# wangheda/youtube-8m

Measured on AMD Instinct MI355X. Metric: training videos/sec, higher is better.
Workload: dtype f32; 1 GPU; BASELINE configs[3]: LstmModel (2 x BasicLSTMCell(1024), dynamic_rnn over F=300) on raw uint8 [B,300,1152] frames + MoeModel head (2 mixtures, V=4716), fp32 training step (fwd+bwd+clip+Adam); per_gpu_batch=128, global_batch=128, frames=300, parallelism=dp1, params=113902808

## Files before the change

### include/yt8m_hip.h

```cpp
#ifndef YT8M_HIP_H
#define YT8M_HIP_H
#include <stdint.h>

#ifdef __cplusplus
extern "C" {
#endif

typedef void* yt8m_stream_t;

enum yt8m_status { YT8M_OK = 0, YT8M_E_BADARG = -1, YT8M_E_SHAPE = -2, YT8M_E_HIP = -3, YT8M_E_RCCL = -4 };
enum yt8m_label_dtype { YT8M_LABEL_U8 = 0, YT8M_LABEL_F32 = 1 };

int yt8m_abi_version(void);
const char* yt8m_last_error(void);
const char* yt8m_built_arch(void);

int yt8m_prof_enable(int on);
int yt8m_prof_reset(void);
int yt8m_prof_get(int family, int64_t* launches, double* total_ms);
int yt8m_prof_get_flops(int family, double* flops);
int yt8m_prof_get_bytes(int family, double* bytes);

int yt8m_probe_mfma_f32(int iters, int blocks, float* sink, yt8m_stream_t stream);
int yt8m_probe_mfma_bf16(int iters, int blocks, int random_operands, float* sink, yt8m_stream_t stream);
// ... 23 lines not shown
                          int64_t workspace_bytes, yt8m_stream_t stream);
int yt8m_gemm_bf16_nt_grouped(int nprob, const yt8m_gemm_problem* probs, void* workspace, int64_t workspace_bytes,
                              yt8m_stream_t stream);
int64_t yt8m_x3_image_bytes(int64_t rows, int64_t K);
int yt8m_x3_split(const float* src, int64_t R, int64_t C, int64_t ld, float scale, void* plain, void* trans, yt8m_stream_t stream);
int yt8m_gemm_x3_nt_grouped(int nprob, const yt8m_gemm_problem* probs, void* workspace, int64_t workspace_bytes,
                            yt8m_stream_t stream);
int yt8m_h2_split(const float* src, int64_t R, int64_t C, int64_t ld, float scale, const float* dscale, void* plain, void* trans,
                  float* colpart, yt8m_stream_t stream);
int yt8m_h2_absmax(const float* src, int64_t R, int64_t C, int64_t ld, void* word, yt8m_stream_t stream);
int yt8m_h2_degraded(uint64_t* counts, int reset, yt8m_stream_t stream);
int yt8m_h2_split_dropout(const float* src, int64_t R, int64_t C, float scale, const float* dscale, void* plain, void* trans,
                          float keep_prob, uint64_t seed, int64_t offset, yt8m_stream_t stream);
int yt8m_h2_split_rowmax(const float* src, int64_t R, int64_t C, int64_t ld, const void* rowmax, float* inv, void* plain,
                         yt8m_stream_t stream);
int yt8m_h2_split_ex(const float* src, int64_t R, int64_t C, int64_t ld, float scale, const void* dscale, const float* rowscale, void* plain,
                     void* trans, void* trans_scaled, float* colpart, float* colpart_scaled, yt8m_stream_t stream);
int yt8m_gemm_h1x2_nt_ex(int64_t M, int64_t N, int64_t K, const void* A1, int64_t ska, const void* B2, int64_t skb, float* C, int64_t ldc,
                         const float* bias, float alpha, const void* dsb, const float* rowscale, const float* colsum, float colsum_scale,
                         float beta, void* workspace, int64_t workspace_bytes, yt8m_stream_t stream);
int yt8m_h2_rowscales(const float* src, int64_t R, int64_t C, int64_t ld, float* S, float* inv, yt8m_stream_t stream);
int yt8m_h2_split_rows(const float* src, int64_t R, int64_t C, int64_t ld, const float* S, void* plain, yt8m_stream_t stream);
int yt8m_gemm_h2_nt_ex(int64_t M, int64_t N, int64_t K, const void* A2, int64_t ska, const void* B2, int64_t skb, float* C, int64_t ldc,
                       const float* bias, float alpha, const void* dsa, const void* dsb, const float* rowscale, float beta, void* workspace,
                       int64_t workspace_bytes, yt8m_stream_t stream);
int yt8m_timepool_max_f32(const float* y, int64_t F, int64_t B, int64_t N, int64_t ldy, float* out, int32_t* idx, int64_t ldo,
                          yt8m_stream_t stream);
int yt8m_timepool_shiftmax_f32(const float* z, int64_t F, int64_t B, int64_t ldz, int nfilt, const int32_t* fs, const int32_t* ncol, float* out,
                               int32_t* idx, int64_t ldo, yt8m_stream_t stream);
int yt8m_u8_cnn_pool_dw(const uint8_t* q, const float* r_tm, const int32_t* idx, const float* g, int64_t ldg, int64_t B, int64_t F, int64_t D,
// ... 282 lines not shown
  int64_t B, F, D, H;
  int32_t L;
  int32_t input_u8;
  float forget_bias;
  int32_t fwd_chunks;
  int32_t bwd_chunks;
  int32_t need_dx;
  float input_keep_prob;
  int32_t reserved0;
  uint64_t dropout_seed[8];
} yt8m_lstm_stack_desc;
int yt8m_lstm_stack_supported(const yt8m_lstm_stack_desc* desc);
int64_t yt8m_lstm_stack_tape_bytes(const yt8m_lstm_stack_desc* desc);
int64_t yt8m_lstm_stack_scratch_bytes(const yt8m_lstm_stack_desc* desc);
int yt8m_lstm_stack_partition(const yt8m_lstm_stack_desc* desc, int* fwd_chunks, int* bwd_chunks);
int yt8m_lstm_stack_streams(int L, yt8m_stream_t* layer_streams, yt8m_stream_t* wgrad_stream);
int yt8m_lstm_stack_fwd(const yt8m_lstm_stack_desc* desc, const void* x, const int32_t* num_frames, const float* const* W,
                        const float* const* b, void* tape, int64_t tape_bytes, void* scratch, int64_t scratch_bytes,
                        yt8m_stream_t stream);
int yt8m_lstm_stack_view(const yt8m_lstm_stack_desc* desc, void* tape, int layer, int which, float** out);
int yt8m_lstm_stack_bwd(const yt8m_lstm_stack_desc* desc, const void* x, const int32_t* num_frames, const float* const* W, void* tape,
                        int64_t tape_bytes, void* scratch, int64_t scratch_bytes, const float* dout_top,
                        const float* const* dc_final, const float* const* dh_final, float* const* dW, float* const* db,
                        const float* beta_W, const float* beta_b, float* dx, yt8m_stream_t stream);
int yt8m_lstm_stack_status(const yt8m_lstm_stack_desc* desc, void* scratch, yt8m_stream_t stream);
int yt8m_lstm_stack_layer_done_wait(int layer, yt8m_stream_t stream);
int yt8m_lstm_stack_use_streams(int set, int* previous);
typedef void (*yt8m_stream_hook)(void* user, yt8m_stream_t stream);
int yt8m_lstm_stack_set_prep_hook(yt8m_stream_hook hook, void* user);
typedef struct yt8m_opt_ranges {
// ... 166 lines not shown
```

### youtube-8m_amd/_lib.py

```python
import ctypes
import os

_HERE = os.path.dirname(os.path.abspath(__file__))
LIB_PATH = os.environ.get("YT8M_LIB", os.path.join(_HERE, "libyt8m_hip.so"))

c_void_p, c_int, c_int64, c_float, c_double = ctypes.c_void_p, ctypes.c_int, ctypes.c_int64, ctypes.c_float, ctypes.c_double
P = c_void_p

class GemmProblem(ctypes.Structure):
    _fields_ = [("M", c_int64), ("N", c_int64), ("K", c_int64), ("A", c_void_p), ("lda", c_int64), ("B", c_void_p),
                ("ldb", c_int64), ("C", c_void_p), ("ldc", c_int64), ("bias", c_void_p), ("beta", c_float)]


STREAM_HOOK = ctypes.CFUNCTYPE(None, ctypes.c_void_p, ctypes.c_void_p)


class PersistBwdImages(ctypes.Structure):
    _fields_ = [("plain", ctypes.c_void_p), ("trans", ctypes.c_void_p), ("trans_scaled", ctypes.c_void_p), ("rowscale", ctypes.c_void_p),
                ("colpart", ctypes.c_void_p), ("colpart_scaled", ctypes.c_void_p)]


class LstmStackDesc(ctypes.Structure):
    _fields_ = [("B", c_int64), ("F", c_int64), ("D", c_int64), ("H", c_int64), ("L", ctypes.c_int32), ("input_u8", ctypes.c_int32),
                ("forget_bias", c_float), ("fwd_chunks", ctypes.c_int32), ("bwd_chunks", ctypes.c_int32), ("need_dx", ctypes.c_int32),
# ... 159 lines not shown
    "yt8m_lstm_persist_set_cus": (c_int, [c_int, c_int]),
    "yt8m_lstm_persist_get_cus": (c_int, [ctypes.POINTER(c_int), ctypes.POINTER(c_int)]),
    "yt8m_lstm_persist_status": (c_int, [P, P]),
    "yt8m_lstm_persist_reserve_cus": (c_int, [c_int, ctypes.POINTER(c_int)]),
    "yt8m_lstm_persist_debug_fault": (c_int, [P, P]),
    "yt8m_lstm_persist_fwd": (c_int, [P, P, c_int64, P, P, P, P, c_int64, c_int64, c_int64, c_int64, c_float, P, c_int64, P]),
    "yt8m_lstm_persist_fwd_bf16": (c_int, [P, P, c_int64, P, P, P, P, c_int64, c_int64, c_int64, c_int64, c_float, P, c_int64, P]),
    "yt8m_lstm_persist_bwd_supported": (c_int, [c_int64, c_int64]),
    "yt8m_lstm_persist_bwd": (c_int, [P, P, c_int64, P, P, P, P, c_int, P, P, c_int64, c_int64, c_int64, c_int64, P, c_int64, P]),
    "yt8m_lstm_persist_bwd_bf16": (c_int, [P, P, c_int64, P, P, P, P, c_int, P, P, c_int64, c_int64, c_int64, c_int64, P, c_int64, P]),
    "yt8m_lstm_persist_fwd_h2": (c_int, [P, P, c_int64, P, P, P, P, c_int64, c_int64, c_int64, c_int64, c_float, P, P, c_int64, P]),
    "yt8m_lstm_persist_bwd_h2": (c_int, [P, P, c_int64, P, P, P, P, c_int, P, P, c_int64, c_int64, c_int64, c_int64, P, P, c_int64, P]),
    "yt8m_lstm_persist_bwd_on_f16_pipe": (c_int, [c_int64, c_int64]),
    "yt8m_lstm_persist_bwd_ex": (c_int, [P, P, c_int64, P, P, P, P, c_int, P, c_int64, c_int64, c_int64, c_int64, P, P, P, P, c_int64, P]),
    "yt8m_h2_split_rowmax": (c_int, [P, c_int64, c_int64, c_int64, P, P, P, P]),
    "yt8m_lstm_persist_bwd_images_rows": (c_int, [c_int64, c_int64]),
    "yt8m_lstm_persist_bwd_images": (c_int, [P, P, c_int64, P, P, P, P, c_int, P, c_int64, c_int64, c_int64, c_int64, P, c_int64, P, P]),
    "yt8m_lstm_packed_floats": (c_int64, [c_int64, c_int64]),
    "yt8m_lstm_pack": (c_int, [P, c_int64, c_int64, P, P, P]),
    "yt8m_lstm_steps_fwd": (c_int, [P, P, c_int64, P, P, P, P, P, c_int64, c_int64, c_int64, c_int64, c_float, P, c_int64, P]),
    "yt8m_lstm_steps_bwd": (c_int, [P, P, c_int64, P, P, P, P, P, c_int, P, c_int64, c_int64, c_int64, c_int64, P, c_int64, P]),
    "yt8m_lstm_layer_bwd": (c_int, [P, P, c_int64, P, P, P, P, P, P, P, c_int64, c_int64, c_int64, P, c_int64, P]),
    "yt8m_attn_softmax_fwd": (c_int, [P, P, P, c_int64, c_int64, c_int64, P]),
    "yt8m_attn_softmax_bwd": (c_int, [P, P, P, P, c_int64, c_int64, c_int64, P]),
    "yt8m_softmax_rows_fwd": (c_int, [P, P, P, c_int64, c_int64, c_int64, P]),
    "yt8m_softmax_rows_bwd": (c_int, [P, P, P, P, c_int64, c_int64, c_int64, P]),
    "yt8m_netvlad_supported": (c_int, [c_int64, c_int64, c_int64, c_int64]),
    "yt8m_netvlad_single_pass": (c_int, [c_int64, c_int64, c_int64, c_int64]),
    "yt8m_netvlad_set_single": (c_int, [c_int]),
    "yt8m_netvlad_workspace_bytes": (c_int64, [c_int64, c_int64, c_int64, c_int64]),
# ... 135 lines not shown
```

### youtube-8m_amd/csrc/gemm_x3.hip

```cpp
#include "common.h"
#include "x3_image.h"
#include "philox.h"
#include <type_traits>
#include <algorithm>
#include <mutex>
#include <stdlib.h>

namespace {

constexpr int TM = 256, TN = 256;
constexpr int PLANE_F = 256 * 8;
constexpr int OP_F = 3 * PLANE_F;
constexpr int NST = 3;
using yt8m_x3::RG_F;
using yt8m_x3::store_block;

typedef float f32x16 __attribute__((ext_vector_type(16)));
typedef __bf16 bf16x8 __attribute__((ext_vector_type(8)));

struct XArgs {
  const float* A;
  const float* B;
  float* C;
  const float* bias;
// ... 1027 lines not shown
        else store_block<NP>(v, trans + ((int64_t)(row >> 5) * KB + kb) * (NP * RG_F), row);
      }
      if (trans_s) {
#pragma unroll
        for (int j = 0; j < 16; ++j) {
          const int r = r0 + blk * 16 + j;
          v[j] *= r < R ? rowscale[r] : 0.f;
        }
        if constexpr (NP == 2) yt8m_x3::store_block_h2(v, trans_s + ((int64_t)(row >> 5) * KB + kb) * (NP * RG_F), row);
        else store_block<NP>(v, trans_s + ((int64_t)(row >> 5) * KB + kb) * (NP * RG_F), row);
      }
    }
  }
}

}

using namespace yt8m;

namespace {
constexpr size_t H2_DEGRADED_BYTES = 256 * 128;
unsigned long long* h2_degraded_words() {
  static std::mutex mu;
  static unsigned long long* words[64] = {};
  static bool tried[64] = {};
  int dev = 0;
  if (hipGetDevice(&dev) != hipSuccess || dev < 0 || dev >= 64) return nullptr;
  std::lock_guard<std::mutex> lk(mu);
  if (!tried[dev]) {
    tried[dev] = true;
// ... 174 lines not shown
                     (float*)nullptr, 1.0f, (const float*)nullptr, (float*)nullptr, (float*)nullptr, (float*)nullptr, (const float*)nullptr, S,
                     (const unsigned*)nullptr, (float*)nullptr, h2_degraded_words());
  return launch_status("x3_split_kernel<2>");
}
extern "C" int yt8m_h2_split_rowmax(const float* src, int64_t R, int64_t C, int64_t ld, const void* rowmax, float* inv, void* plain,
                                    yt8m_stream_t stream) {
  YT8M_REQUIRE(src && rowmax && inv && plain && R >= 1 && C >= 1 && ld >= C && R < (1LL << 31) && C < (1LL << 31), YT8M_E_BADARG, "bad arguments");
  YT8M_REQUIRE((reinterpret_cast<uintptr_t>(plain) & 15) == 0, YT8M_E_BADARG, "images must be 16-byte aligned");
  dim3 grid((unsigned)((C + 63) / 64), (unsigned)((R + 63) / 64));
  YT8M_REQUIRE(grid.y < 65536, YT8M_E_BADARG, "too many rows for one split launch");
  ProfScope prof(F_ELEMENTWISE, as_stream(stream));
  hipLaunchKernelGGL(x3_split_kernel<2>, grid, dim3(256), 0, as_stream(stream), src, ld, (int)R, (int)C, static_cast<float*>(plain),
                     (float*)nullptr, 1.0f, (const float*)nullptr, (float*)nullptr, (float*)nullptr, (float*)nullptr, (const float*)nullptr,
                     (const float*)nullptr, static_cast<const unsigned*>(rowmax), inv, h2_degraded_words());
  return launch_status("x3_split_kernel<2>");
}
extern "C" int yt8m_gemm_h2_nt_ex(int64_t M, int64_t N, int64_t K, const void* A2, int64_t ska, const void* B2, int64_t skb, float* C,
                                  int64_t ldc, const float* bias, float alpha, const void* dsa, const void* dsb, const float* rowscale,
                                  float beta, void* workspace, int64_t workspace_bytes, yt8m_stream_t stream);

extern "C" int yt8m_h2_absmax(const float* src, int64_t R, int64_t C, int64_t ld, void* word, yt8m_stream_t stream) {
  YT8M_REQUIRE(src && word && R >= 1 && C >= 1 && ld >= C && R < (1LL << 31) && C < (1LL << 31), YT8M_E_BADARG, "bad arguments");
  const int64_t n = R * C;
  const unsigned blocks = (unsigned)std::min<int64_t>(2048, (n + 4095) / 4096);
  ProfScope prof(F_ELEMENTWISE, as_stream(stream));
  hipLaunchKernelGGL(h2_absmax_kernel, dim3(blocks), dim3(256), 0, as_stream(stream), src, ld, (int)R, (int)C, static_cast<unsigned*>(word));
  return launch_status("h2_absmax_kernel");
}

extern "C" int yt8m_x3_split_ex(const float* src, int64_t R, int64_t C, int64_t ld, float scale, const float* rowscale, void* plain,
// ... 281 lines not shown
```

### youtube-8m_amd/csrc/lstm_stack.hip

```cpp
#include <stdlib.h>
#include <algorithm>
#include <mutex>
#include <vector>
#include "common.h"

using namespace yt8m;

namespace {

constexpr int MAXL = 8, MAXP = 64;
constexpr int MAXBP = 62;
constexpr float U8_ALPHA = 4.0f / 255.0f;
constexpr float U8_BETA = 128.0f * (4.0f / 255.0f) + (4.0f / 512.0f - 2.0f);
constexpr int64_t X3_MIN_ROWS = 1024;
constexpr int64_t STEP_IMAGES_MAX_BYTES = 8LL << 30;
constexpr float H2_S = 8192.0f;

int64_t up256(int64_t v) { return (v + 255) / 256 * 256; }

int knob(const char* name, int dflt) { const char* v = getenv(name); return v ? atoi(v) : dflt; }

struct Part { int64_t t0, T; };
int chunks(int64_t F, int n, Part* out) {
  if (n < 1) n = 1;
// ... 7 lines not shown

struct Plan {
  int64_t B, F, D, H, FB;
  int L, u8, need_dx;
  int bf16;
  int nf, nb;
  Part fp[MAXP], bp[MAXP];
  int64_t z[MAXL], cs[MAXL], hs[MAXL], out[MAXL], rrow, tape_bytes;
  int64_t pws[MAXL], pws_bytes;
  int64_t gws[MAXL + 1], gws_bytes;
  int64_t gwx[MAXL], gws2;
  int64_t qimg, w3t, wcs, wxt3[MAXL], xi[MAXL];
  int64_t dz[MAXL], dbuf[MAXL], work[MAXL];
  int64_t dz3[MAXL], wx3[MAXL], dzT3[MAXL], dzT3s, csr, dbdummy;
  int64_t xT[MAXL], hT[MAXL];
  int64_t cpart[MAXL], cparts;
  bool colparts;
  int img_rows;
  int h2;
  int64_t hsc;
  int64_t hx0;
  int64_t hrow, hrow_stride;
  float keep;
  uint64_t seed[MAXL];
  int emit_max;
  int64_t rmax, rmax_stride;
  int64_t cimg[MAXL], cimgs;
  int64_t scratch_bytes;
};

// ... 62 lines not shown
  p.pws_bytes = up256(pb);
  o = 0;
  for (int l = 0; l < p.L; ++l) { p.pws[l] = o; o += p.pws_bytes; }
  p.gws_bytes = up256(yt8m_gemm_workspace_bytes());
  for (int l = 0; l <= p.L; ++l) { p.gws[l] = o; o += p.gws_bytes; }
  for (int l = 0; l < p.L; ++l) { p.gwx[l] = o; o += p.gws_bytes; }
  p.gws2 = o; o += p.gws_bytes;
  auto ib = [&](int64_t rows, int64_t K) { return p.bf16 ? x1_bytes(rows, K) : x3_bytes(rows, K); };
  const int64_t H4 = 4 * p.H;
  p.qimg = o; o += p.u8 ? up256(x1_bytes(p.FB, p.D)) : 0;
  p.w3t = o; o += p.u8 ? up256(ib(H4, p.D)) : 0;
  p.wcs = o; o += up256(H4 * 4);
  int64_t fmax = 0, bmax = 0;
  for (int c = 0; c < p.nf; ++c) fmax = std::max(fmax, p.fp[c].T * p.B);
  for (int c = 0; c < p.nb; ++c) bmax = std::max(bmax, p.bp[c].T * p.B);
  for (int l = 0; l < p.L; ++l) {
    const int64_t Din = l ? p.H : p.D;
    const bool x1 = l == 0 && p.u8;
    p.wxt3[l] = o; o += x1 ? 0 : up256(ib(H4, Din));
    p.xi[l] = o; o += x1 ? 0 : up256(ib(fmax, Din));
    p.dz[l] = o; o += up256(FBH * 4 * 4);
    p.dbuf[l] = o; o += l + 1 < p.L ? up256(FBH * 4) : 0;
    p.work[l] = o; o += up256(4 * BH * 4);
    const bool dxl = l > 0 || p.need_dx;
    p.dz3[l] = o; o += dxl ? up256(ib(bmax, H4)) : 0;
    p.wx3[l] = o; o += dxl ? up256(ib(Din, H4)) : 0;
    p.xT[l] = o; o += x1 ? up256(x1_bytes(p.D, p.FB)) : up256(ib(Din, p.FB));
    p.hT[l] = o; o += up256(ib(p.H, p.FB));
  }
  p.h2 = (knob("YT8M_STACK_H2", 1) && !p.bf16) ? 1 : 0;
  p.keep = (d->input_keep_prob > 0.f && d->input_keep_prob < 1.f) ? d->input_keep_prob : 0.f;
  for (int l = 0; l < MAXL; ++l) p.seed[l] = d->dropout_seed[l];
  if (d->input_keep_prob < 0.f || d->input_keep_prob > 1.f) return "input_keep_prob must be in [0, 1]";
  if (p.keep > 0.f && (p.u8 || !p.h2 || p.keep < 0.3f || (p.D % 4) != 0 || (p.H % 4) != 0))
    return "input dropout: float input, f16 product forms (YT8M_STACK_H2), keep_prob >= 0.3, D % 4 == 0";
  p.img_rows = (knob("YT8M_STACK_FUSED_IMAGES", 0) && !p.bf16 && !p.h2) ? yt8m_lstm_persist_bwd_images_rows(p.B, p.H) : 0;
  const int64_t trows = p.img_rows ? p.FB : bmax;
  for (int l = 0; l < p.L; ++l) { p.dzT3[l] = o; o += up256(ib(H4, trows)); }
  p.dzT3s = o; o += p.u8 ? up256(ib(H4, trows)) : 0;
  const int64_t ci = p.img_rows ? up256((int64_t)p.img_rows * MAXP * 2 * H4 * 4) : 0;
  for (int l = 0; l < p.L; ++l) { p.cimg[l] = o; o += ci; }
  p.cimgs = o; o += p.u8 ? ci : 0;
  p.csr = o; o += up256(H4 * 4);
  p.dbdummy = o; o += up256(H4 * 4);
  p.hsc = o; o += 256 * MAXL;
  p.hx0 = o; o += 256;
  p.hrow_stride = up256(bmax * 4);
  p.hrow = o; o += p.h2 ? p.hrow_stride * 2 * MAXL : 0;
  p.emit_max = (p.h2 && knob("YT8M_STACK_DZ_MAXIMA", 1) && yt8m_lstm_persist_bwd_images_rows(p.B, p.H) > 0 && per_step && p.nb <= 61) ? 1 : 0;
  p.rmax_stride = up256(p.FB * 4);
  p.rmax = o; o += p.emit_max ? p.rmax_stride * p.L : 0;
  p.colparts = knob("YT8M_STACK_COLPARTS", 1) != 0;
  for (int c = 0; c < p.nb; ++c) p.colparts = p.colparts && (p.bp[c].t0 * p.B) % 64 == 0 && (p.bp[c].T * p.B) % 64 == 0;
  const int64_t cp = p.colparts ? up256(((p.FB + 63) / 64) * H4 * 4) : 0;
  for (int l = 0; l < p.L; ++l) { p.cpart[l] = o; o += cp; }
  p.cparts = o; o += p.u8 ? cp : 0;
  p.scratch_bytes = o;
  return nullptr;
}

struct DevState {
  hipStream_t rs[MAXL] = {nullptr};
  hipStream_t dxs[MAXL] = {nullptr};
  hipStream_t sw = nullptr, sw2 = nullptr;
// ... 76 lines not shown
}

extern "C" int yt8m_lstm_stack_supported(const yt8m_lstm_stack_desc* desc) {
  Plan P;
  const char* why = plan(desc, &P);
  if (why) { snprintf(g_err, sizeof(g_err), "yt8m_lstm_stack: %s", why); return 0; }
  return 1;
}
extern "C" int64_t yt8m_lstm_stack_tape_bytes(const yt8m_lstm_stack_desc* desc) {
  Plan P;
  return plan(desc, &P) ? 0 : P.tape_bytes;
}
extern "C" int64_t yt8m_lstm_stack_scratch_bytes(const yt8m_lstm_stack_desc* desc) {
  Plan P;
  return plan(desc, &P) ? 0 : P.scratch_bytes;
}
extern "C" int yt8m_lstm_stack_partition(const yt8m_lstm_stack_desc* desc, int* fwd_chunks, int* bwd_chunks) {
  Plan P;
  const char* why = plan(desc, &P);
  YT8M_REQUIRE(!why, YT8M_E_SHAPE, why ? why : "");
  if (fwd_chunks) *fwd_chunks = P.nf;
  if (bwd_chunks) *bwd_chunks = P.nb;
  return YT8M_OK;
}

extern "C" int yt8m_lstm_stack_streams(int L, yt8m_stream_t* layer_streams, yt8m_stream_t* wgrad_stream) {
  YT8M_REQUIRE(L >= 1 && L <= MAXL && layer_streams, YT8M_E_BADARG, "1..8 layers, non-null output");
  std::lock_guard<std::mutex> lk(g_mu);
  DevState* S = nullptr;
  RC(dev_state(L, &S));
// ... 260 lines not shown
    return bf ? yt8m_bf16_image(src, R, C, ld, scale, plain, trans, (yt8m_stream_t)st) : yt8m_x3_split(src, R, C, ld, scale, plain, trans, (yt8m_stream_t)st);
  };
  auto gemm = [&](int n, const yt8m_gemm_problem* pr, void* ws, int64_t wsb, hipStream_t st) {
    return bf ? yt8m_gemm_b1_nt_grouped(n, pr, ws, wsb, (yt8m_stream_t)st) : yt8m_gemm_x3_nt_grouped(n, pr, ws, wsb, (yt8m_stream_t)st);
  };
  hipEvent_t start = ev.record(main);
  ev.wait(sw, start);
  if (two_sw) ev.wait(S->sw2, start);
  for (int l = 0; l < P.L; ++l) { ev.wait(S->rs[l], start); if (dx_stream) ev.wait(S->dxs[l], start); }
  if (P.h2)
    for (int l = 0; l < P.L; ++l) {
      YT8M_HIP_CHECK(hipMemsetAsync(at<char>(scratch, P.hsc + 256 * l + 4), 0, 248, S->rs[l]));
      if (P.emit_max && l >= 1) YT8M_HIP_CHECK(hipMemsetAsync(at<char>(scratch, P.rmax + l * P.rmax_stride), 0, (size_t)FB * 4, S->rs[l]));
    }
  for (int l = 0; l < P.L; ++l) {
    if (!dW[l]) continue;
    if (l == 0 && P.u8) {
      if (P.h2) RC(yt8m_u8_frames_image_t_f16(static_cast<const uint8_t*>(x), num_frames, B, P.F, D, at<char>(scratch, P.xT[0]), sw));
      else RC(yt8m_u8_frames_image_t(static_cast<const uint8_t*>(x), num_frames, B, P.F, D, at<char>(scratch, P.xT[0]), sw));
    } else {
      const float* src = l ? at<float>(tape, P.out[l - 1]) : static_cast<const float*>(x);
      const int64_t Din = l ? H : D;
      if (P.h2 && P.keep > 0.f)
        RC(yt8m_h2_split_dropout(src, FB, Din, l ? H2_S : 1.0f, l ? nullptr : at<float>(scratch, P.hx0), nullptr, at<char>(scratch, P.xT[l]),
                                 P.keep, P.seed[l], 0, (yt8m_stream_t)sw));
      else if (P.h2 && l >= 1) RC(yt8m_h2_split(src, FB, Din, Din, H2_S, nullptr, nullptr, at<char>(scratch, P.xT[l]), nullptr, (yt8m_stream_t)sw));
      else if (P.h2) RC(yt8m_h2_split(src, FB, Din, Din, 1.0f, at<float>(scratch, P.hx0), nullptr, at<char>(scratch, P.xT[0]), nullptr, (yt8m_stream_t)sw));
      else RC(split(src, FB, Din, Din, 1.0f, nullptr, at<char>(scratch, P.xT[l]), sw));
    }
    if (P.h2) RC(yt8m_h2_split(at<float>(tape, P.hs[l]), FB, H, H, H2_S, nullptr, nullptr, at<char>(scratch, P.hT[l]), nullptr, (yt8m_stream_t)sw));
    else RC(split(at<float>(tape, P.hs[l]), FB, H, H, 1.0f, nullptr, at<char>(scratch, P.hT[l]), sw));
  }
  yt8m_stream_hook hook = g_prep_hook;
  void* hook_user = g_prep_user;
  g_prep_hook = nullptr;
  g_prep_user = nullptr;
  bool early = g_early.set;
  g_early.set = false;
  if (two_sw) ev.wait(S->sw2, ev.record(sw));
  int phase[MAXL];
  bool wx3_done[MAXL];
  const void* wx_img[MAXL] = {nullptr};
  hipEvent_t dzT_free[MAXL] = {nullptr};
  const bool fused_img = P.img_rows > 0 && !dx_stream && !fuse_dz;
  int64_t img_done_rows[MAXL] = {0};
  int img_launches[MAXL] = {0};
  for (int l = 0; l < P.L; ++l) {
    hipStream_t s = S->rs[l];
    float* work = at<float>(scratch, P.work[l]);
    const float* dh = dh_final ? dh_final[l] : nullptr;
    const float* dc = dc_final ? dc_final[l] : nullptr;
    if (dh) YT8M_HIP_CHECK(hipMemcpyAsync(work, dh, (size_t)BH * 4, hipMemcpyDeviceToDevice, s));
    else YT8M_HIP_CHECK(hipMemsetAsync(work, 0, (size_t)BH * 4, s));
    if (dc) YT8M_HIP_CHECK(hipMemcpyAsync(work + BH, dc, (size_t)BH * 4, hipMemcpyDeviceToDevice, s));
    else YT8M_HIP_CHECK(hipMemsetAsync(work + BH, 0, (size_t)BH * 4, s));
    phase[l] = 0;
    wx3_done[l] = false;
  }
// ... 65 lines not shown
            nullptr, num_frames, t0, T, B, H, at<char>(scratch, P.pws[l]), P.pws_bytes, s));
      }
      phase[l] = (int)((phase[l] + T) % 2);
      hipEvent_t rb = ev.record(s);
      if (hook) {
        hook(hook_user, (yt8m_stream_t)S->sw);
        hook = nullptr;
      }
      if (early) {
        early = false;
        RC(yt8m_optimizer_ranges(&g_early.o, (yt8m_stream_t)S->sw));
      }
      bool fused_t = false;
      const float* dzc = dz + t0 * B * H4;
      if (j == nsub - 1) dx_ev = nullptr;
      if (l > 0 || P.need_dx) {
        hipStream_t sx = dx_stream ? S->dxs[l] : s;
        if (dx_stream) ev.wait(sx, rb);
        fused_t = fuse_dz && dW[l] && !(l == 0 && P.u8);
        if (fused_t && dzT_free[l]) ev.wait(sx, dzT_free[l]);
        static const int h2_dx_knob = knob("YT8M_STACK_H2_DX", 1);
        const bool dx_h2 = P.h2 && l >= 1 && h2_dx_knob;
        if (dx_h2) {
          float* rS = at<float>(scratch, P.hrow + 2 * l * P.hrow_stride);
          float* rI = at<float>(scratch, P.hrow + (2 * l + 1) * P.hrow_stride);
          if (P.emit_max) {
            RC(yt8m_h2_split_rowmax(dzc, M, H4, H4, at<char>(scratch, P.rmax + l * P.rmax_stride + t0 * B * 4), rI, at<char>(scratch, P.dz3[l]),
                                    (yt8m_stream_t)sx));
          } else {
            RC(yt8m_h2_rowscales(dzc, M, H4, H4, rS, rI, (yt8m_stream_t)sx));
            RC(yt8m_h2_split_rows(dzc, M, H4, H4, rS, at<char>(scratch, P.dz3[l]), (yt8m_stream_t)sx));
          }
          const float* wword = at<float>(scratch, P.hsc + 256 * l);
          if (!wx3_done[l]) {
            RC(yt8m_h2_split(W[l], Din, H4, H4, 1.0f, wword, at<char>(scratch, P.wx3[l]), nullptr, nullptr, (yt8m_stream_t)sx));
            wx3_done[l] = true;
          }
          float* dst = at<float>(scratch, P.dbuf[l - 1]) + t0 * B * H;
          RC(yt8m_gemm_h2_nt_ex(M, Din, H4, at<char>(scratch, P.dz3[l]), 0, at<char>(scratch, P.wx3[l]), 0, dst, Din, nullptr, 1.0f, nullptr,
                                wword, rI, 0.0f, at<char>(scratch, dx_stream ? P.gwx[l] : P.gws[l]), P.gws_bytes, (yt8m_stream_t)sx));
          if (P.keep > 0.f)
// ... 28 lines not shown
      ev.wait(sw, rb);
      void* gw = at<char>(scratch, (two_sw && l == 0) ? P.gws2 : P.gws[P.L]);
      const float bW = first ? (beta_W ? beta_W[l] : 0.f) : 1.f;
      const bool lastpart = c == 0 && j == 0;
      if (dW[l]) {
        if (l == 0 && P.u8 && P.h2) {
          const float* rr = at<float>(tape, P.rrow) + t0 * B;
          float* word = at<float>(scratch, P.hsc) + 1 + c;
          if (!P.emit_max) RC(yt8m_h2_absmax(dzc, M, H4, H4, word, (yt8m_stream_t)sw));
          float* cp = P.colparts ? at<float>(scratch, P.cpart[l]) + (t0 * B / 64) * H4 : nullptr;
          float* cps = P.colparts ? at<float>(scratch, P.cparts) + (t0 * B / 64) * H4 : nullptr;
          RC(yt8m_h2_split_ex(dzc, M, H4, H4, 1.0f, word, rr, nullptr, at<char>(scratch, P.dzT3[l]), at<char>(scratch, P.dzT3s), cp, cps,
                              (yt8m_stream_t)sw));
          RC(yt8m_gemm_h1x2_nt_ex(D, H4, M, at<char>(scratch, P.xT[0]) + kb0 * 1024, KBtot, at<char>(scratch, P.dzT3s), 0, dW[0], H4, nullptr,
                                  U8_ALPHA, word, nullptr, nullptr, 0.f, bW, gw, P.gws_bytes, (yt8m_stream_t)sw));
          yt8m_gemm_problem pr = {H, H4, M, at<char>(scratch, P.hT[0]) + kb0 * 2048, KBtot, at<char>(scratch, P.dzT3[l]), 0,
                                  dW[0] + D * H4, H4, nullptr, bW};
          const float alpha = 1.0f / H2_S;
          const float* dsb = word;
          RC(yt8m_gemm_h2_nt_grouped(1, &pr, &alpha, nullptr, &dsb, gw, P.gws_bytes, (yt8m_stream_t)sw));
        } else if (l == 0 && P.u8) {
          const float* rr = at<float>(tape, P.rrow) + t0 * B;
          if (fused_img) {
          } else if (P.colparts || bf) {
            float* cp = P.colparts ? at<float>(scratch, P.cpart[l]) + (t0 * B / 64) * H4 : nullptr;
            float* cps = P.colparts ? at<float>(scratch, P.cparts) + (t0 * B / 64) * H4 : nullptr;
            if (bf) RC(yt8m_bf16_image_colsum(dzc, M, H4, H4, 1.0f, rr, nullptr, at<char>(scratch, P.dzT3[l]), at<char>(scratch, P.dzT3s), cp, cps, sw));
            else RC(yt8m_x3_split_colsum(dzc, M, H4, H4, 1.0f, rr, nullptr, at<char>(scratch, P.dzT3[l]), at<char>(scratch, P.dzT3s), cp, cps, sw));
          } else
            RC(yt8m_x3_split_ex(dzc, M, H4, H4, 1.0f, rr, nullptr, at<char>(scratch, P.dzT3[l]), at<char>(scratch, P.dzT3s), sw));
          if (bf)
            RC(yt8m_gemm_b1_nt_ex(D, H4, M, at<char>(scratch, P.xT[0]) + kb0 * 1024, KBtot, dzTs_img, 0, dW[0], H4,
                                  nullptr, U8_ALPHA, nullptr, nullptr, 0.f, bW, gw, P.gws_bytes, sw));
          else
            RC(yt8m_gemm_x1x3_nt_ex(D, H4, M, at<char>(scratch, P.xT[0]) + kb0 * 1024, KBtot, dzTs_img, 0, dW[0], H4,
                                    nullptr, U8_ALPHA, nullptr, nullptr, 0.f, bW, gw, P.gws_bytes, sw));
          yt8m_gemm_problem pr = {H, H4, M, at<char>(scratch, P.hT[0]) + kb0 * KBB, KBtot, dzT_img, 0,
                                  dW[0] + D * H4, H4, nullptr, bW};
          RC(gemm(1, &pr, gw, P.gws_bytes, sw));
        } else if (P.h2) {
          float* word = at<float>(scratch, P.hsc + 256 * l) + 1 + c;
          if (!P.emit_max) RC(yt8m_h2_absmax(dzc, M, H4, H4, word, (yt8m_stream_t)sw));
          float* cp = (P.colparts && db[l]) ? at<float>(scratch, P.cpart[l]) + (t0 * B / 64) * H4 : nullptr;
          RC(yt8m_h2_split(dzc, M, H4, H4, 1.0f, word, nullptr, at<char>(scratch, P.dzT3[l]), cp, (yt8m_stream_t)sw));
          yt8m_gemm_problem pr[2] = {
              {Din, H4, M, at<char>(scratch, P.xT[l]) + kb0 * 2048, KBtot, at<char>(scratch, P.dzT3[l]), 0, dW[l], H4, nullptr, bW},
              {H, H4, M, at<char>(scratch, P.hT[l]) + kb0 * 2048, KBtot, at<char>(scratch, P.dzT3[l]), 0, dW[l] + Din * H4, H4, nullptr, bW}};
          const float alphas[2] = {l ? 1.0f / H2_S : 1.0f, 1.0f / H2_S};
          const float* dsa[2] = {l ? nullptr : at<float>(scratch, P.hx0), nullptr};
          const float* dsb[2] = {word, word};
          RC(yt8m_gemm_h2_nt_grouped(2, pr, alphas, dsa, dsb, gw, P.gws_bytes, (yt8m_stream_t)sw));
        } else {
          if (fused_img) {
          } else if (!fused_t) {
            if (P.colparts && db[l]) {
              float* cp = at<float>(scratch, P.cpart[l]) + (t0 * B / 64) * H4;
              if (bf) RC(yt8m_bf16_image_colsum(dzc, M, H4, H4, 1.0f, nullptr, nullptr, at<char>(scratch, P.dzT3[l]), nullptr, cp, nullptr, sw));
              else RC(yt8m_x3_split_colsum(dzc, M, H4, H4, 1.0f, nullptr, nullptr, at<char>(scratch, P.dzT3[l]), nullptr, cp, nullptr, sw));
            } else {
              RC(split(dzc, M, H4, H4, 1.0f, nullptr, at<char>(scratch, P.dzT3[l]), sw));
            }
          }
          yt8m_gemm_problem pr[2] = {
              {Din, H4, M, at<char>(scratch, P.xT[l]) + kb0 * KBB, KBtot, dzT_img, 0, dW[l], H4, nullptr, bW},
              {H, H4, M, at<char>(scratch, P.hT[l]) + kb0 * KBB, KBtot, dzT_img, 0, dW[l] + Din * H4, H4, nullptr, bW}};
          RC(gemm(2, pr, gw, P.gws_bytes, sw));
// ... 38 lines not shown
```

Before: 8128 videos/s.

## Share transposed hidden-state images across LSTM layers and add dual dz split kernel

When the shared-HT mode applies (h2 path, no dropout, L>=2, B%16==0), layer l-1's transposed h image is extended by B rows so it doubles as layer l's input image. Layer l>=1 therefore no longer builds or stores its own xT image, which removes one split pass and its scratch per layer. The change also adds an optional fused kernel that writes the row-scaled plain dz image and the transposed dz image in one pass, with double-buffered event handoff. The fused kernel is off by default (DZ_DUAL=0) while shared-HT is on by default. This adds stride and offset complexity to the weight-gradient GEMMs.

```diff
diff --git a/include/yt8m_hip.h b/include/yt8m_hip.h
--- a/include/yt8m_hip.h
+++ b/include/yt8m_hip.h
@@ -61,6 +61,8 @@
                           float keep_prob, uint64_t seed, int64_t offset, yt8m_stream_t stream);
 int yt8m_h2_split_rowmax(const float* src, int64_t R, int64_t C, int64_t ld, const void* rowmax, float* inv, void* plain,
                          yt8m_stream_t stream);
+int yt8m_h2_split_dual(const float* src, int64_t R, int64_t C, int64_t ld, const void* rowmax, const void* dscale, float* inv, void* plain,
+                       void* trans, float* colpart, yt8m_stream_t stream);
 int yt8m_h2_split_ex(const float* src, int64_t R, int64_t C, int64_t ld, float scale, const void* dscale, const float* rowscale, void* plain,
                      void* trans, void* trans_scaled, float* colpart, float* colpart_scaled, yt8m_stream_t stream);
 int yt8m_gemm_h1x2_nt_ex(int64_t M, int64_t N, int64_t K, const void* A1, int64_t ska, const void* B2, int64_t skb, float* C, int64_t ldc,
@@ -373,6 +375,7 @@
 int64_t yt8m_lstm_stack_tape_bytes(const yt8m_lstm_stack_desc* desc);
 int64_t yt8m_lstm_stack_scratch_bytes(const yt8m_lstm_stack_desc* desc);
 int yt8m_lstm_stack_partition(const yt8m_lstm_stack_desc* desc, int* fwd_chunks, int* bwd_chunks);
+int yt8m_lstm_stack_image_forms(const yt8m_lstm_stack_desc* desc, int* shared_ht, int* dz_dual);
 int yt8m_lstm_stack_streams(int L, yt8m_stream_t* layer_streams, yt8m_stream_t* wgrad_stream);
 int yt8m_lstm_stack_fwd(const yt8m_lstm_stack_desc* desc, const void* x, const int32_t* num_frames, const float* const* W,
                         const float* const* b, void* tape, int64_t tape_bytes, void* scratch, int64_t scratch_bytes,
diff --git a/youtube-8m_amd/_lib.py b/youtube-8m_amd/_lib.py
--- a/youtube-8m_amd/_lib.py
+++ b/youtube-8m_amd/_lib.py
@@ -197,6 +197,8 @@
     "yt8m_lstm_persist_bwd_on_f16_pipe": (c_int, [c_int64, c_int64]),
     "yt8m_lstm_persist_bwd_ex": (c_int, [P, P, c_int64, P, P, P, P, c_int, P, c_int64, c_int64, c_int64, c_int64, P, P, P, P, c_int64, P]),
     "yt8m_h2_split_rowmax": (c_int, [P, c_int64, c_int64, c_int64, P, P, P, P]),
+    "yt8m_h2_split_dual": (c_int, [P, c_int64, c_int64, c_int64, P, P, P, P, P, P, P]),
+    "yt8m_lstm_stack_image_forms": (c_int, [P, P, P]),
     "yt8m_lstm_persist_bwd_images_rows": (c_int, [c_int64, c_int64]),
     "yt8m_lstm_persist_bwd_images": (c_int, [P, P, c_int64, P, P, P, P, c_int, P, c_int64, c_int64, c_int64, c_int64, P, c_int64, P, P]),
     "yt8m_lstm_packed_floats": (c_int64, [c_int64, c_int64]),
diff --git a/youtube-8m_amd/csrc/gemm_x3.hip b/youtube-8m_amd/csrc/gemm_x3.hip
--- a/youtube-8m_amd/csrc/gemm_x3.hip
+++ b/youtube-8m_amd/csrc/gemm_x3.hip
@@ -1065,6 +1065,89 @@
   }
 }
 
+__global__ __launch_bounds__(256) void h2_split_dual_kernel(const float* __restrict__ src, int64_t ld, int R, int Cc, float* __restrict__ plain,
+                                                            float* __restrict__ trans, float* __restrict__ colpart,
+                                                            const unsigned* __restrict__ dscale, const unsigned* __restrict__ rowmaxw,
+                                                            float* __restrict__ rowinv, unsigned long long* __restrict__ degraded) {
+  __shared__ float T[64][65];
+  __shared__ float RS[64];
+  const float ts = yt8m_x3::pow2_scale_for(__uint_as_float(dscale[0]), 14);
+  const int r0 = blockIdx.y * 64, c0 = blockIdx.x * 64;
+  const int t = threadIdx.x;
+  unsigned n_clamp = 0, n_flush = 0;
+  {
+    const int c4 = (t & 15) * 4, rr = t >> 4;
+    const bool vec = (ld & 3) == 0 && (reinterpret_cast<uintptr_t>(src) & 15) == 0;
+#pragma unroll
+    for (int i = 0; i < 4; ++i) {
+      const int r = rr + 16 * i;
+      float4 v = {0.f, 0.f, 0.f, 0.f};
+      float pr = 1.f;
+      if (r0 + r < R) {
+        const float* p = src + (int64_t)(r0 + r) * ld + c0 + c4;
+        if (vec && c0 + c4 + 3 < Cc) v = *reinterpret_cast<const float4*>(p);
+        else {
+          if (c0 + c4 + 0 < Cc) v.x = p[0];
+          if (c0 + c4 + 1 < Cc) v.y = p[1];
+          if (c0 + c4 + 2 < Cc) v.z = p[2];
+          if (c0 + c4 + 3 < Cc) v.w = p[3];
+        }
+        pr = yt8m_x3::pow2_scale_for(__uint_as_float(rowmaxw[r0 + r]), 14);
+        if (rowinv && blockIdx.x == 0 && (t & 15) == 0) rowinv[r0 + r] = 1.0f / pr;
+      }
+      if ((t & 15) == 0) RS[r] = pr;
+      T[r][c4 + 0] = v.x; T[r][c4 + 1] = v.y; T[r][c4 + 2] = v.z; T[r][c4 + 3] = v.w;
+#ifndef YT8M_H2_NO_COUNT
+      const float sv[8] = {v.x * pr, v.y * pr, v.z * pr, v.w * pr, v.x * ts, v.y * ts, v.z * ts, v.w * ts};
+#pragma unroll
+      for (int e = 0; e < 8; ++e) {
+        const float m = fabsf(sv[e]);
+        n_clamp += (m > 65504.f && m < 3.0e38f) ? 1u : 0u;
+        n_flush += (m != 0.f && m < 2.98023224e-8f) ? 1u : 0u;
+      }
+#endif
+    }
+  }
+  if (degraded && __any((n_clamp | n_flush) != 0u)) {
+#pragma unroll
+    for (int o = 32; o > 0; o >>= 1) { n_clamp += __shfl_xor(n_clamp, o, 64); n_flush += __shfl_xor(n_flush, o, 64); }
+    if ((t & 63) == 0) {
+      unsigned long long* w = degraded + (size_t)((blockIdx.x + blockIdx.y * 7u + (unsigned)(t >> 6) * 61u) & 255u) * 16;
+      if (n_clamp) atomicAdd(w, (unsigned long long)n_clamp);
+      if (n_flush) atomicAdd(w + 1, (unsigned long long)n_flush);
+    }
+  }
+  __syncthreads();
+  if (colpart && t < 64 && c0 + t < Cc) {
+    float acc = 0.f;
+    for (int r = 0; r < 64; ++r) acc += __fmul_rn(T[r][t], ts);
+    acc *= 1.0f / ts;
+    colpart[(int64_t)blockIdx.y * Cc + c0 + t] = acc;
+  }
+  const int a = t & 63, blk = t >> 6;
+  {
+    const int KB = (Cc + 15) >> 4;
+    const int row = r0 + a, kb = (c0 >> 4) + blk;
+    if (row < ((R + 31) & ~31) && kb < KB) {
+      const float s = RS[a];
+      float v[16];
+#pragma unroll
+      for (int j = 0; j < 16; ++j) v[j] = T[a][blk * 16 + j] * s;
+      yt8m_x3::store_block_h2(v, plain + ((int64_t)(row >> 5) * KB + kb) * (2 * RG_F), row);
+    }
+  }
+  {
+    const int KB = (R + 15) >> 4;
+    const int row = c0 + a, kb = (r0 >> 4) + blk;
+    if (row < ((Cc + 31) & ~31) && kb < KB) {
+      float v[16];
+#pragma unroll
+      for (int j = 0; j < 16; ++j) v[j] = T[blk * 16 + j][a] * ts;
+      yt8m_x3::store_block_h2(v, trans + ((int64_t)(row >> 5) * KB + kb) * (2 * RG_F), row);
+    }
+  }
+}
+
 }
 
 using namespace yt8m;
@@ -1269,6 +1352,20 @@
                      (float*)nullptr, 1.0f, (const float*)nullptr, (float*)nullptr, (float*)nullptr, (float*)nullptr, (const float*)nullptr,
                      (const float*)nullptr, static_cast<const unsigned*>(rowmax), inv, h2_degraded_words());
   return launch_status("x3_split_kernel<2>");
+}
+extern "C" int yt8m_h2_split_dual(const float* src, int64_t R, int64_t C, int64_t ld, const void* rowmax, const void* dscale, float* inv,
+                                  void* plain, void* trans, float* colpart, yt8m_stream_t stream) {
+  YT8M_REQUIRE(src && rowmax && dscale && inv && plain && trans && R >= 1 && C >= 1 && ld >= C && R < (1LL << 31) && C < (1LL << 31),
+               YT8M_E_BADARG, "bad arguments");
+  YT8M_REQUIRE(((reinterpret_cast<uintptr_t>(plain) | reinterpret_cast<uintptr_t>(trans)) & 15) == 0, YT8M_E_BADARG,
+               "images must be 16-byte aligned");
+  dim3 grid((unsigned)((C + 63) / 64), (unsigned)((R + 63) / 64));
+  YT8M_REQUIRE(grid.y < 65536, YT8M_E_BADARG, "too many rows for one split launch");
+  ProfScope prof(F_ELEMENTWISE, as_stream(stream));
+  hipLaunchKernelGGL(h2_split_dual_kernel, grid, dim3(256), 0, as_stream(stream), src, ld, (int)R, (int)C, static_cast<float*>(plain),
+                     static_cast<float*>(trans), colpart, static_cast<const unsigned*>(dscale), static_cast<const unsigned*>(rowmax), inv,
+                     h2_degraded_words());
+  return launch_status("h2_split_dual_kernel");
 }
 extern "C" int yt8m_gemm_h2_nt_ex(int64_t M, int64_t N, int64_t K, const void* A2, int64_t ska, const void* B2, int64_t skb, float* C,
                                   int64_t ldc, const float* bias, float alpha, const void* dsa, const void* dsb, const float* rowscale,
diff --git a/youtube-8m_amd/csrc/lstm_stack.hip b/youtube-8m_amd/csrc/lstm_stack.hip
--- a/youtube-8m_amd/csrc/lstm_stack.hip
+++ b/youtube-8m_amd/csrc/lstm_stack.hip
@@ -45,6 +45,10 @@
   int64_t dz[MAXL], dbuf[MAXL], work[MAXL];
   int64_t dz3[MAXL], wx3[MAXL], dzT3[MAXL], dzT3s, csr, dbdummy;
   int64_t xT[MAXL], hT[MAXL];
+  int shared_ht;
+  int64_t hTkb[MAXL];
+  int dz_dual;
+  int64_t dzT3b[MAXL];
   int64_t cpart[MAXL], cparts;
   bool colparts;
   int img_rows;
@@ -137,6 +141,9 @@
   int64_t fmax = 0, bmax = 0;
   for (int c = 0; c < p.nf; ++c) fmax = std::max(fmax, p.fp[c].T * p.B);
   for (int c = 0; c < p.nb; ++c) bmax = std::max(bmax, p.bp[c].T * p.B);
+  p.h2 = (knob("YT8M_STACK_H2", 1) && !p.bf16) ? 1 : 0;
+  p.keep = (d->input_keep_prob > 0.f && d->input_keep_prob < 1.f) ? d->input_keep_prob : 0.f;
+  p.shared_ht = (p.h2 && p.keep == 0.f && p.L >= 2 && p.B % 16 == 0 && knob("YT8M_STACK_SHARED_HT", 1)) ? 1 : 0;
   for (int l = 0; l < p.L; ++l) {
     const int64_t Din = l ? p.H : p.D;
     const bool x1 = l == 0 && p.u8;
@@ -148,11 +155,11 @@
     const bool dxl = l > 0 || p.need_dx;
     p.dz3[l] = o; o += dxl ? up256(ib(bmax, H4)) : 0;
     p.wx3[l] = o; o += dxl ? up256(ib(Din, H4)) : 0;
-    p.xT[l] = o; o += x1 ? up256(x1_bytes(p.D, p.FB)) : up256(ib(Din, p.FB));
-    p.hT[l] = o; o += up256(ib(p.H, p.FB));
-  }
-  p.h2 = (knob("YT8M_STACK_H2", 1) && !p.bf16) ? 1 : 0;
-  p.keep = (d->input_keep_prob > 0.f && d->input_keep_prob < 1.f) ? d->input_keep_prob : 0.f;
+    p.xT[l] = o; o += x1 ? up256(x1_bytes(p.D, p.FB)) : (p.shared_ht && l >= 1) ? 0 : up256(ib(Din, p.FB));
+    const int64_t hrows = (p.shared_ht && l + 1 < p.L) ? p.FB + p.B : p.FB;
+    p.hTkb[l] = hrows / 16;
+    p.hT[l] = o; o += up256(ib(p.H, hrows));
+  }
   for (int l = 0; l < MAXL; ++l) p.seed[l] = d->dropout_seed[l];
   if (d->input_keep_prob < 0.f || d->input_keep_prob > 1.f) return "input_keep_prob must be in [0, 1]";
   if (p.keep > 0.f && (p.u8 || !p.h2 || p.keep < 0.3f || (p.D % 4) != 0 || (p.H % 4) != 0))
@@ -171,6 +178,9 @@
   p.hrow_stride = up256(bmax * 4);
   p.hrow = o; o += p.h2 ? p.hrow_stride * 2 * MAXL : 0;
   p.emit_max = (p.h2 && knob("YT8M_STACK_DZ_MAXIMA", 1) && yt8m_lstm_persist_bwd_images_rows(p.B, p.H) > 0 && per_step && p.nb <= 61) ? 1 : 0;
+  p.dz_dual = (p.emit_max && p.L >= 2 && knob("YT8M_STACK_H2_DX", 1) && !knob("YT8M_STACK_DX_STREAM", 0)) ? knob("YT8M_STACK_DZ_DUAL", 0) : 0;
+  if (p.dz_dual < 0 || p.dz_dual > 2) p.dz_dual = 0;
+  for (int l = 0; l < p.L; ++l) { p.dzT3b[l] = o; o += (p.dz_dual == 1 && l >= 1) ? up256(ib(H4, bmax)) : 0; }
   p.rmax_stride = up256(p.FB * 4);
   p.rmax = o; o += p.emit_max ? p.rmax_stride * p.L : 0;
   p.colparts = knob("YT8M_STACK_COLPARTS", 1) != 0;
@@ -277,6 +287,14 @@
 extern "C" int64_t yt8m_lstm_stack_scratch_bytes(const yt8m_lstm_stack_desc* desc) {
   Plan P;
   return plan(desc, &P) ? 0 : P.scratch_bytes;
+}
+extern "C" int yt8m_lstm_stack_image_forms(const yt8m_lstm_stack_desc* desc, int* shared_ht, int* dz_dual) {
+  Plan P;
+  const char* why = plan(desc, &P);
+  YT8M_REQUIRE(!why, YT8M_E_SHAPE, why ? why : "");
+  if (shared_ht) *shared_ht = P.shared_ht;
+  if (dz_dual) *dz_dual = P.dz_dual;
+  return YT8M_OK;
 }
 extern "C" int yt8m_lstm_stack_partition(const yt8m_lstm_stack_desc* desc, int* fwd_chunks, int* bwd_chunks) {
   Plan P;
@@ -567,8 +585,10 @@
       if (P.emit_max && l >= 1) YT8M_HIP_CHECK(hipMemsetAsync(at<char>(scratch, P.rmax + l * P.rmax_stride), 0, (size_t)FB * 4, S->rs[l]));
     }
   for (int l = 0; l < P.L; ++l) {
-    if (!dW[l]) continue;
-    if (l == 0 && P.u8) {
+    const bool x_shared = P.shared_ht && l >= 1;
+    const bool h_wanted = dW[l] || (P.shared_ht && l + 1 < P.L && dW[l + 1]);
+    if (!dW[l] || x_shared) {
+    } else if (l == 0 && P.u8) {
       if (P.h2) RC(yt8m_u8_frames_image_t_f16(static_cast<const uint8_t*>(x), num_frames, B, P.F, D, at<char>(scratch, P.xT[0]), sw));
       else RC(yt8m_u8_frames_image_t(static_cast<const uint8_t*>(x), num_frames, B, P.F, D, at<char>(scratch, P.xT[0]), sw));
     } else {
@@ -581,7 +601,9 @@
       else if (P.h2) RC(yt8m_h2_split(src, FB, Din, Din, 1.0f, at<float>(scratch, P.hx0), nullptr, at<char>(scratch, P.xT[0]), nullptr, (yt8m_stream_t)sw));
       else RC(split(src, FB, Din, Din, 1.0f, nullptr, at<char>(scratch, P.xT[l]), sw));
     }
-    if (P.h2) RC(yt8m_h2_split(at<float>(tape, P.hs[l]), FB, H, H, H2_S, nullptr, nullptr, at<char>(scratch, P.hT[l]), nullptr, (yt8m_stream_t)sw));
+    if (!h_wanted) continue;
+    if (P.h2)
+      RC(yt8m_h2_split(at<float>(tape, P.hs[l]), P.hTkb[l] * 16, H, H, H2_S, nullptr, nullptr, at<char>(scratch, P.hT[l]), nullptr, (yt8m_stream_t)sw));
     else RC(split(at<float>(tape, P.hs[l]), FB, H, H, 1.0f, nullptr, at<char>(scratch, P.hT[l]), sw));
   }
   yt8m_stream_hook hook = g_prep_hook;
@@ -595,6 +617,8 @@
   bool wx3_done[MAXL];
   const void* wx_img[MAXL] = {nullptr};
   hipEvent_t dzT_free[MAXL] = {nullptr};
+  hipEvent_t dualT_free[MAXL][2] = {{nullptr}};
+  int dual_n[MAXL] = {0};
   const bool fused_img = P.img_rows > 0 && !dx_stream && !fuse_dz;
   int64_t img_done_rows[MAXL] = {0};
   int img_launches[MAXL] = {0};
@@ -690,6 +714,8 @@
       bool fused_t = false;
       const float* dzc = dz + t0 * B * H4;
       if (j == nsub - 1) dx_ev = nullptr;
+      const int dual = (l >= 1 && dW[l]) ? P.dz_dual : 0;
+      char* dzT_h2 = at<char>(scratch, (dual == 1 && (dual_n[l] & 1)) ? P.dzT3b[l] : P.dzT3[l]);
       if (l > 0 || P.need_dx) {
         hipStream_t sx = dx_stream ? S->dxs[l] : s;
         if (dx_stream) ev.wait(sx, rb);
@@ -700,7 +726,18 @@
         if (dx_h2) {
           float* rS = at<float>(scratch, P.hrow + 2 * l * P.hrow_stride);
           float* rI = at<float>(scratch, P.hrow + (2 * l + 1) * P.hrow_stride);
-          if (P.emit_max) {
+          if (dual) {
+            hipStream_t sd = dual == 2 ? S->sw : sx;
+            hipEvent_t& freed = dualT_free[l][dual_n[l] & 1];
+            if (dual == 2) ev.wait(sd, rb);
+            else if (freed) ev.wait(sd, freed);
+            float* cp = (P.colparts && db[l]) ? at<float>(scratch, P.cpart[l]) + (t0 * B / 64) * H4 : nullptr;
+            RC(yt8m_h2_split_dual(dzc, M, H4, H4, at<char>(scratch, P.rmax + l * P.rmax_stride + t0 * B * 4),
+                                  at<char>(scratch, P.hsc + 256 * l + 4 * (1 + c)), rI, at<char>(scratch, P.dz3[l]), dzT_h2, cp, (yt8m_stream_t)sd));
+            hipEvent_t made = ev.record(sd);
+            if (dual == 2) ev.wait(sx, made);
+            else rb = made;
+          } else if (P.emit_max) {
             RC(yt8m_h2_split_rowmax(dzc, M, H4, H4, at<char>(scratch, P.rmax + l * P.rmax_stride + t0 * B * 4), rI, at<char>(scratch, P.dz3[l]),
                                     (yt8m_stream_t)sx));
           } else {
@@ -759,7 +796,7 @@
                               (yt8m_stream_t)sw));
           RC(yt8m_gemm_h1x2_nt_ex(D, H4, M, at<char>(scratch, P.xT[0]) + kb0 * 1024, KBtot, at<char>(scratch, P.dzT3s), 0, dW[0], H4, nullptr,
                                   U8_ALPHA, word, nullptr, nullptr, 0.f, bW, gw, P.gws_bytes, (yt8m_stream_t)sw));
-          yt8m_gemm_problem pr = {H, H4, M, at<char>(scratch, P.hT[0]) + kb0 * 2048, KBtot, at<char>(scratch, P.dzT3[l]), 0,
+          yt8m_gemm_problem pr = {H, H4, M, at<char>(scratch, P.hT[0]) + kb0 * 2048, P.hTkb[0], at<char>(scratch, P.dzT3[l]), 0,
                                   dW[0] + D * H4, H4, nullptr, bW};
           const float alpha = 1.0f / H2_S;
           const float* dsb = word;
@@ -786,15 +823,21 @@
         } else if (P.h2) {
           float* word = at<float>(scratch, P.hsc + 256 * l) + 1 + c;
           if (!P.emit_max) RC(yt8m_h2_absmax(dzc, M, H4, H4, word, (yt8m_stream_t)sw));
-          float* cp = (P.colparts && db[l]) ? at<float>(scratch, P.cpart[l]) + (t0 * B / 64) * H4 : nullptr;
-          RC(yt8m_h2_split(dzc, M, H4, H4, 1.0f, word, nullptr, at<char>(scratch, P.dzT3[l]), cp, (yt8m_stream_t)sw));
+          if (!dual) {
+            float* cp = (P.colparts && db[l]) ? at<float>(scratch, P.cpart[l]) + (t0 * B / 64) * H4 : nullptr;
+            RC(yt8m_h2_split(dzc, M, H4, H4, 1.0f, word, nullptr, dzT_h2, cp, (yt8m_stream_t)sw));
+          }
+          const bool x_shared = P.shared_ht && l >= 1;
+          const char* xa = x_shared ? at<char>(scratch, P.hT[l - 1]) + (kb0 + B / 16) * 2048 : at<char>(scratch, P.xT[l]) + kb0 * 2048;
           yt8m_gemm_problem pr[2] = {
-              {Din, H4, M, at<char>(scratch, P.xT[l]) + kb0 * 2048, KBtot, at<char>(scratch, P.dzT3[l]), 0, dW[l], H4, nullptr, bW},
-              {H, H4, M, at<char>(scratch, P.hT[l]) + kb0 * 2048, KBtot, at<char>(scratch, P.dzT3[l]), 0, dW[l] + Din * H4, H4, nullptr, bW}};
+              {Din, H4, M, xa, x_shared ? P.hTkb[l - 1] : KBtot, dzT_h2, 0, dW[l], H4, nullptr, bW},
+              {H, H4, M, at<char>(scratch, P.hT[l]) + kb0 * 2048, P.hTkb[l], dzT_h2, 0, dW[l] + Din * H4, H4, nullptr, bW}};
           const float alphas[2] = {l ? 1.0f / H2_S : 1.0f, 1.0f / H2_S};
           const float* dsa[2] = {l ? nullptr : at<float>(scratch, P.hx0), nullptr};
           const float* dsb[2] = {word, word};
           RC(yt8m_gemm_h2_nt_grouped(2, pr, alphas, dsa, dsb, gw, P.gws_bytes, (yt8m_stream_t)sw));
+          if (dual == 1) dualT_free[l][dual_n[l] & 1] = ev.record(sw);
+          if (dual) ++dual_n[l];
         } else {
           if (fused_img) {
           } else if (!fused_t) {
```

Result: no change. 8175 videos/s, median of 6 (+0.6%).
